# TimHarrelson/QuantumSimulations

Measured on AMD Instinct MI355X. Metric: detuning-points/hour (N=14 sea-detuning sweep, 3 variants per point), higher is better.
Workload: dtype f64 (complex128 state); 1 GPU; config 3: n_sea=13+1 rare (N=14 qubits), one 64-point sweep split over 1 GPU(s) (64 detunings in [0,150 kHz] x 3 variants = 192 evolutions on rank 0), t_final=0.001s, 101 outputs, 7 observables; propagator=exact Chebyshev (tol 1e-14), engine_mode=persistent, outputs_per_launch=2, parallelism=evolution-sharded x1 (strong scaling, no collectives), span_problems=0

## Files before the change

quantumsimulations_amd/csrc/dse_interval.hip:

```cpp
#include <type_traits>

#include "dse_device.h"

namespace dse {

#ifdef DSE_DIAG
__device__ int g_dse_ablate_iv = 0;
hipError_t set_ablate_interval(int mask) {
  return hipMemcpyToSymbol(HIP_SYMBOL(g_dse_ablate_iv), &mask, sizeof(int));
}
#else
constexpr int g_dse_ablate_iv = 0;
hipError_t set_ablate_interval(int mask) { return mask ? hipErrorNotSupported : hipSuccess; }
#endif

namespace {

typedef __attribute__((address_space(1))) int gint;


template <bool IMAG>
__device__ __forceinline__ double2 dmad(double2 acc, double cr, double ci, double2 s) {
  if (IMAG) {
    acc.x = fma(-ci, s.y, acc.x);
    acc.y = fma(ci, s.x, acc.y);
    return acc;
  }
  return cmad(acc, cr, ci, s);
}

__device__ __forceinline__ void rmad(double2& acc, double g, double2 s) {
  acc.x = fma(g, s.x, acc.x);
  acc.y = fma(g, s.y, acc.y);
}

typedef __attribute__((address_space(3))) const dv2 ldv2;

template <typename T>
__device__ __forceinline__ uint32_t lds_addr(const T* p) {
  return (uint32_t)(size_t)(const __attribute__((address_space(3))) T*)p;
}

template <int NT, int NH, int NR>
__device__ __forceinline__ void ld_rows(const double2* w, int t, int hh, int r0, double2* v) {
  uint32_t a = lds_addr(w + t);
  constexpr uint32_t HALF = (uint32_t)NH * NT * 16u;
  if (hh) {
    if (HALF >= 65536u)
      asm("v_add_u32_e32 %0, %1, %2" : "=v"(a) : "i"(HALF), "v"(a));
    else
      a += HALF;
  }
#pragma unroll
  for (int rr = 0; rr < NR; ++rr) {
    const dv2 d = *(ldv2*)(size_t)(a + (uint32_t)(r0 + rr) * NT * 16u);
    v[rr] = make_double2(d.x, d.y);
  }
}

template <int L>
struct IvShared {
  double2 w[RB<L>::T];
  double c[L + 1];
  double zz[L * L];
  double zr[kRegAmps];
  dv2 td[3][RB<L>::NT];
  double xg[kRegBits];
  double xq[RB<L>::TB];
  dv2 it[RB<L>::TB][8];
};

template <int L, bool IMAG>
__global__ void __launch_bounds__(RB<L>::NT)
k_interval(const DevProb* __restrict__ probs, const int2* __restrict__ items, int q, int set,
           int n_out, int* __restrict__ flags, int* __restrict__ err, HandoffKnobs hk, long colstride) {
  constexpr int NT = RB<L>::NT, R = kRegAmps, TB = RB<L>::TB, NH = R / 2;
  constexpr bool PIPE = DSE_PIPE && IMAG;
  constexpr uint32_t T = 1u << L;
  __shared__ IvShared<L> S;
  __shared__ int s_fail;

  if (__hip_atomic_load(err, __ATOMIC_RELAXED, __HIP_MEMORY_SCOPE_AGENT) != 0) return;
  const int2 it = items[blockIdx.x];
  const DevProb& P = probs[it.x];
  const uint32_t h = colstride ? 0u : (uint32_t)it.y;
  const size_t coff = colstride ? (size_t)it.y * (size_t)colstride : 0;
  const int tid = threadIdx.x;
  const bool pair = (P.n == L + 1);
  const bool xgen = pair && P.n_pairs_hi > 0;
  const int K = P.degree;
  const double s1 = P.s1;
  const uint32_t b_me = h & 1u, b_pa = b_me ^ 1u;

  constexpr uint32_t TBYTES = T * 16u;
  const __amdgpu_buffer_rsrc_t psi_me = tile_rsrc(P.buf[q ? 2 : 0] + coff + (h << L), TBYTES);
  const __amdgpu_buffer_rsrc_t psi_pa = tile_rsrc(P.buf[q ? 2 : 0] + ((h ^ 1u) << L), TBYTES);
  double2* const xs_me = P.xslots + ((size_t)h * kXSlots << L);
  double2* const xs_pa = P.xslots + ((size_t)(h ^ 1u) * kXSlots << L);
  const __amdgpu_buffer_rsrc_t acc_t = tile_rsrc(P.buf[q ? 0 : 2] + coff + (h << L), TBYTES);
  const uint32_t voff = (uint32_t)tid * 16u;
  const int lane = tid & 63;
  const int wave = __builtin_amdgcn_readfirstlane(tid >> 6);
  gint* flag_me = (gint*)flags + (2 * it.x + (int)h) * kIvWaves + wave;
  const gint* flag_pa = (const gint*)flags + (2 * it.x + (int)(h ^ 1u)) * kIvWaves + wave;

  const cptr<DPair> cph = cst(P.pairs_hi);
  const cptr<DFlip> cfh = cst(P.flips_hi);
  const double* crow = (const double*)coef_row(P, set, 0);
  const size_t rstride = 2 * (size_t)(P.kcap1 + 1);
  int dj[kMaxOut];
#pragma unroll
  for (int j = 0; j < kMaxOut; ++j) dj[j] = j < n_out ? (int)crow[j * rstride] : 0;

  const int ab = g_dse_ablate_iv;
  const bool fences = hk.fences != 0;

  if (tid == 0) s_fail = 0;
  {
    const gdbl* zz = gptr(P.zz);
    const int n = P.n;
    for (int e = tid; e < L * L; e += NT) {
      const int i = e / L, j = e % L;
      S.zz[e] = (j > i) ? zz[i * n + j] : 0.0;
    }
    tile_diag_coeffs<L>(P, h, P.beta, S.c, tid);
    static_assert(sizeof(DSweep) == 80 && sizeof(DPair) == 16, "iteration table layout");
    const gd2* psw = (const gd2*)P.sweeps;
    const gd2* ptt = (const gd2*)P.pairs_tt;
    for (int e = tid; e < 8 * TB; e += NT) {
      const int j = e >> 3, c = e & 7;
      dv2 v;
      v.x = v.y = 0.0;
      if (c < 4)
        v = psw[j * 5 + c];
      else if (4 * j + c - 4 < P.n_pairs_tt)
        v = ptt[4 * j + c - 4];
      S.it[j][c] = v;
    }
  }
#pragma unroll
  for (int r = 0; r < R; ++r) S.w[r * NT + tid] = bld(psi_me, voff, (uint32_t)(r * NT * 16));
  __syncthreads();
  if (tid < kRegAmps) {
    double v = 0.0;
    for (int a = 0; a < kRegBits; ++a)
      for (int b = a + 1; b < kRegBits; ++b)
        v += S.zz[(TB + a) * L + TB + b] * ((0.5 - ((tid >> a) & 1)) * (0.5 - ((tid >> b) & 1)));
    S.zr[tid] = v;
  }
  double zt = S.c[L];
  double hr[kRegBits];
#pragma unroll
  for (int i = 0; i < kRegBits; ++i) hr[i] = S.c[TB + i];
#pragma unroll 1
  for (int j = 0; j < TB; ++j) {
    const double sj = 0.5 - (double)((tid >> j) & 1);
    double a = S.c[j];
#pragma unroll 1
    for (int i = j + 1; i < TB; ++i) a += S.zz[j * L + i] * (0.5 - (double)((tid >> i) & 1));
    zt += a * sj;
#pragma unroll
    for (int i = 0; i < kRegBits; ++i) hr[i] += S.zz[j * L + TB + i] * sj;
  }
  static_assert(kRegBits == 4, "td packing");
  {
    dv2 v;
    v.x = zt, v.y = hr[0];
    S.td[0][tid] = v;
    v.x = hr[1], v.y = hr[2];
    S.td[1][tid] = v;
    v.x = hr[3], v.y = 0.0;
    S.td[2][tid] = v;
  }
  if (tid < kRegBits) {
    double g = 0.0;
    if (xgen)
      for (int p = 0; p < P.n_pairs_hi; ++p)
        if (cph[p].mask_lo == (1u << (TB + tid))) g = cph[p].g;
    S.xg[tid] = g;
  }
  if (tid < TB) {
    double g = 0.0;
    if (xgen)
      for (int p = 0; p < P.n_pairs_hi; ++p)
        if (cph[p].mask_lo == (1u << tid)) g = cph[p].g;
    S.xq[tid] = g;
  }
  __syncthreads();

  double2 prev[R];
#pragma unroll
  for (int r = 0; r < R; ++r) prev[r] = make_double2(0.0, 0.0);

  auto term_loop = [&](auto xg_tag) {
  constexpr bool xgen = decltype(xg_tag)::value;
  const bool xraw = pair && !xgen;
  for (int k = 1; k <= K; ++k) {
    double2 out[R];
    auto phase1 = [&]() {
      double2 own[R];
#pragma unroll
      for (int r = 0; r < R; ++r) own[r] = S.w[r * NT + tid];
      if (ab & (512 | 4)) {
#pragma unroll
        for (int r = 0; r < R; ++r) out[r] = own[r];
      } else {
        const dv2 t01 = S.td[0][tid], t23 = S.td[1][tid], t4 = S.td[2][tid];
        const double tdv[1 + kRegBits] = {t01.x, t01.y, t23.x, t23.y, t4.x};
#pragma unroll
        for (int r = 0; r < R; ++r) {
          double d = tdv[0] + S.zr[r];
#pragma unroll
          for (int i = 0; i < kRegBits; ++i) d += ((r >> i) & 1 ? -0.5 : 0.5) * tdv[1 + i];
          out[r].x = d * own[r].x;
          out[r].y = d * own[r].y;
        }
        if (P.rflip_mask) {
#pragma unroll
          for (int i = 0; i < kRegBits; ++i) {
            if (!((P.rflip_mask >> i) & 1)) continue;
            const double c0r = P.rflip[i][0], c0i = P.rflip[i][1], c1r = P.rflip[i][2], c1i = P.rflip[i][3];
#pragma unroll
            for (int r = 0; r < R; ++r) {
              const bool v = (r >> i) & 1;
              out[r] = dmad<IMAG>(out[r], v ? c1r : c0r, v ? c1i : c0i, own[r ^ (1 << i)]);
            }
          }
        }
#pragma unroll
        for (int a = 0; a < kRegBits; ++a)
#pragma unroll
          for (int b = a + 1; b < kRegBits; ++b) {
            const double g = P.rr_g[rr_index(a, b)];
            if (g == 0.0) continue;
#pragma unroll
            for (int r = 0; r < R; ++r) {
              if (((r >> a) ^ (r >> b)) & 1) continue;
              rmad(out[r], g, own[r ^ ((1 << a) | (1 << b))]);
            }
          }
      }
    };
    if constexpr (!xgen) phase1();
    __syncthreads();

    if (xgen && !(ab & 64)) {
      double2 u[R];
#pragma unroll
      for (int r = 0; r < R; ++r) u[r] = make_double2(0.0, 0.0);
#pragma unroll
      for (int hh = 0; hh < 2; ++hh) {
        double2 ow[NH];
        ld_rows<NT, NH, NH>(S.w, tid, hh, 0, ow);
        for (int f = 0; f < P.n_flips_hi; ++f) {
          const double cr = b_pa ? cfh[f].re1 : cfh[f].re0, ci = b_pa ? cfh[f].im1 : cfh[f].im0;
#pragma unroll
          for (int rr = 0; rr < NH; ++rr) u[hh * NH + rr] = cmad(u[hh * NH + rr], cr, ci, ow[rr]);
        }
#pragma unroll
        for (int i = 0; i < 3; ++i)
#pragma unroll
          for (int rr = 0; rr < NH; ++rr) {
            const double g = (((rr >> i) & 1u) == b_pa) ? S.xg[i] : 0.0;
            rmad(u[hh * NH + rr], g, ow[rr ^ (1 << i)]);
          }
        {
          const double g = ((uint32_t)(1 - hh) == b_pa) ? S.xg[3] : 0.0;
#pragma unroll
          for (int rr = 0; rr < NH; ++rr) rmad(u[(1 - hh) * NH + rr], g, ow[rr]);
        }
      }
      constexpr int JL = TB < 6 ? TB : 6;
      double2 ba[NH], bb[NH];
      ld_rows<NT, NH, NH>(S.w, tid ^ 1, 0, 0, ba);
#pragma unroll
      for (int j = 0; j < JL; ++j) {
        const double gj = ((uint32_t)((tid >> j) & 1) == b_pa) ? S.xq[j] : 0.0;
        ld_rows<NT, NH, NH>(S.w, tid ^ (1 << j), 1, 0, bb);
#pragma unroll
        for (int rr = 0; rr < NH; ++rr) rmad(u[rr], gj, ba[rr]);
        if (j + 1 < JL) ld_rows<NT, NH, NH>(S.w, tid ^ (1 << (j + 1)), 0, 0, ba);
#pragma unroll
        for (int rr = 0; rr < NH; ++rr) rmad(u[NH + rr], gj, bb[rr]);
      }
#pragma unroll
      for (int j = JL; j < TB; ++j) {
        if ((uint32_t)__builtin_amdgcn_readfirstlane((tid >> j) & 1) != b_pa) continue;
        const double gj = S.xq[j];
        ld_rows<NT, NH, NH>(S.w, tid ^ (1 << j), 0, 0, ba);
        ld_rows<NT, NH, NH>(S.w, tid ^ (1 << j), 1, 0, bb);
#pragma unroll
        for (int rr = 0; rr < NH; ++rr) rmad(u[rr], gj, ba[rr]);
#pragma unroll
        for (int rr = 0; rr < NH; ++rr) rmad(u[NH + rr], gj, bb[rr]);
      }
      const __amdgpu_buffer_rsrc_t dst = tile_rsrc(xs_me + ((size_t)((k - 1) % kXSlots) << L), TBYTES);
#pragma unroll
      for (int r = 0; r < R; ++r) bst<kSc1>(dst, voff, (uint32_t)(r * NT * 16), u[r]);
    }

    if constexpr (xgen) phase1();

    auto publish = [&]() {
      if (pair && !(ab & 64) && (xgen || k > 1)) {
        asm volatile("s_waitcnt vmcnt(0)" ::: "memory");
        if (lane == 0) {
          if (fences) {
            __builtin_amdgcn_fence(__ATOMIC_RELEASE, "agent");
            asm volatile("s_waitcnt vmcnt(0)" ::: "memory");
          }
          __hip_atomic_store(flag_me, k, __ATOMIC_RELAXED, __HIP_MEMORY_SCOPE_AGENT);
        }
      }
    };

    constexpr int J_PUB = TB / 2;

#pragma unroll 1
    for (int j = 0; j < ((ab & 512) ? 0 : TB); ++j) {
      if (j == J_PUB) publish();
      const int pt = tid ^ (1 << j);
      double2 pv[NH];
      if constexpr (PIPE) ld_rows<NT, NH, NH>(S.w, pt, 0, 0, pv);
      dv2 swv[4], ttv[4];
      {
        uint32_t ia;
        asm("v_mov_b32_e32 %0, %1" : "=v"(ia) : "s"(lds_addr(&S.it[j][0])));
#pragma unroll
        for (int e = 0; e < 4; ++e) swv[e] = *(ldv2*)(size_t)(ia + 16u * e);
#pragma unroll
        for (int e = 0; e < 4; ++e) ttv[e] = *(ldv2*)(size_t)(ia + 16u * (4 + e));
      }
      const int bj = (tid >> j) & 1;
      const double cr = bj ? swv[1].x : swv[0].x, ci = bj ? swv[1].y : swv[0].y;
      double g0[kRegBits], g1[kRegBits];
#pragma unroll
      for (int i = 0; i < kRegBits; ++i) {
        const double g = (i & 1) ? swv[2 + i / 2].y : swv[2 + i / 2].x;
        g0[i] = bj ? 0.0 : g;
        g1[i] = bj ? g : 0.0;
      }
      int tpt[4];
      double ge[4];
#pragma unroll
      for (int qq = 0; qq < 4; ++qq) {
        const uint32_t m = (uint32_t)__double_as_longlong(ttv[qq].x);
        tpt[qq] = tid ^ (int)m;
        ge[qq] = par32((uint32_t)tid & m) ? 0.0 : ttv[qq].y;
      }
      auto gsel = [&](int i, int bit) { return bit ? g1[i] : g0[i]; };
      auto sweep = [&](int hh, const double2* pv) {
        double2* oh = out + hh * NH;
#pragma unroll
        for (int rr = 0; rr < NH; ++rr) oh[rr] = dmad<IMAG>(oh[rr], cr, ci, pv[rr]);
#pragma unroll
        for (int i = 0; i < 3; ++i)
#pragma unroll
          for (int rr = 0; rr < NH; ++rr) rmad(oh[rr], gsel(i, (rr >> i) & 1), pv[rr ^ (1 << i)]);
        double2* oo = out + (1 - hh) * NH;
        const double g3 = gsel(3, 1 - hh);
#pragma unroll
        for (int rr = 0; rr < NH; ++rr) rmad(oo[rr], g3, pv[rr]);
      };
      auto tpair = [&](int qq, int hh, const double2* tv) {
        double2* oh = out + hh * NH;
#pragma unroll
        for (int rr = 0; rr < NH; ++rr) rmad(oh[rr], ge[qq], tv[rr]);
      };
      if constexpr (PIPE) {
        constexpr int NQ = NH / 2;
        auto tpair_q = [&](int qq, int hh, int qh, const double2* tv) {
          double2* oh = out + hh * NH + qh * NQ;
#pragma unroll
          for (int rr = 0; rr < NQ; ++rr) rmad(oh[rr], ge[qq], tv[rr]);
        };
        double2 qa[NQ], qb[NQ];
#pragma unroll
        for (int hh = 0; hh < 2; ++hh) {
          ld_rows<NT, NH, NQ>(S.w, tpt[0], hh, 0, qa);
          sweep(hh, pv);
#pragma unroll
          for (int qq = 0; qq < 4; ++qq) {
            ld_rows<NT, NH, NQ>(S.w, tpt[qq], hh, NQ, qb);
            tpair_q(qq, hh, 0, qa);
            if (qq < 3)
              ld_rows<NT, NH, NQ>(S.w, tpt[qq + 1], hh, 0, qa);
            else if (hh == 0)
              ld_rows<NT, NH, NH>(S.w, pt, 1, 0, pv);
            tpair_q(qq, hh, 1, qb);
          }
        }
      } else {
#pragma unroll
        for (int hh = 0; hh < 2; ++hh) {
          ld_rows<NT, NH, NH>(S.w, pt, hh, 0, pv);
          sweep(hh, pv);
#pragma unroll
          for (int qq = 0; qq < 4; ++qq) {
            double2 tv[NH];
            ld_rows<NT, NH, NH>(S.w, tpt[qq], hh, 0, tv);
            tpair(qq, hh, tv);
          }
        }
      }
    }
    if (ab & 512) publish();
    if (pair && !(ab & 128)) {
      const __amdgpu_buffer_rsrc_t src =
          (xraw && k == 1) ? psi_pa : tile_rsrc(xs_pa + ((size_t)((k - 1) % kXSlots) << L), TBYTES);
      double xr = 0.0, xi = 0.0;
      if (xraw && P.n_flips_hi > 0) {
        xr = b_me ? cfh[0].re1 : cfh[0].re0;
        xi = b_me ? cfh[0].im1 : cfh[0].im0;
      }
        if ((xgen || k > 1) && lane == 0 && !(ab & 64)) {
          int spins = 0;
          const int limit = hk.spin_limit;
          while (limit < 0 || __hip_atomic_load(flag_pa, __ATOMIC_RELAXED, __HIP_MEMORY_SCOPE_AGENT) < k) {
            __builtin_amdgcn_s_sleep(1);
            if (limit < 0 || ++spins > limit ||
                ((spins & 1023) == 0 && __hip_atomic_load(err, __ATOMIC_RELAXED, __HIP_MEMORY_SCOPE_AGENT))) {
              s_fail = 1;
              atomicExch(err, 1);
              break;
            }
          }
          if (fences) {
            __builtin_amdgcn_fence(__ATOMIC_ACQUIRE, "agent");
            asm volatile("s_waitcnt vmcnt(0)" ::: "memory");
          }
        }
      asm volatile("" ::: "memory");
#pragma unroll
      for (int hh = 0; hh < 2; ++hh) {
        double2 uv[NH];
#pragma unroll
        for (int rr = 0; rr < NH; ++rr) uv[rr] = bld<kSc1>(src, voff, (uint32_t)((hh * NH + rr) * NT * 16));
#pragma unroll
        for (int rr = 0; rr < NH; ++rr) {
          double2& o = out[hh * NH + rr];
          if (xgen) {
            o.x += uv[rr].x;
            o.y += uv[rr].y;
          } else {
            o = dmad<IMAG>(o, xr, xi, uv[rr]);
          }
        }
      }
    }

#pragma unroll
    for (int r = 0; r < R; ++r) {
      if (k == 1) {
        out[r].x *= s1;
        out[r].y *= s1;
      } else {
        out[r].x = fma(2.0 * s1, out[r].x, -prev[r].x);
        out[r].y = fma(2.0 * s1, out[r].y, -prev[r].y);
      }
    }
    constexpr int AB = kMaxOut <= 2 ? 4 : (kMaxOut == 3 ? 2 : 1);
    const int nj = (ab & 256) ? 0 : n_out;
    bool upd[kMaxOut];
    __amdgpu_buffer_rsrc_t acc_j[kMaxOut];
#pragma unroll
    for (int j = 0; j < kMaxOut; ++j) {
      upd[j] = j < nj && coef_nterm(k, dj[j]) > 0;
      acc_j[j] = (j == n_out - 1) ? acc_t
                                  : tile_rsrc(P.xacc + ((size_t)(q * P.xacc_q + j) << (L + P.tbl)) + (h << L), TBYTES);
    }
#pragma unroll
    for (int r0 = 0; r0 < R; r0 += AB) {
      double2 ownb[AB];
#pragma unroll
      for (int r = 0; r < AB; ++r) ownb[r] = S.w[(r0 + r) * NT + tid];
      double2 accv[kMaxOut][AB];
#pragma unroll
      for (int j = 0; j < kMaxOut; ++j)
        if (upd[j] && k > 1) {
#pragma unroll
          for (int r = 0; r < AB; ++r) accv[j][r] = bld(acc_j[j], voff, (uint32_t)((r0 + r) * NT * 16));
        }
#pragma unroll
      for (int j = 0; j < kMaxOut; ++j) {
        if (!upd[j]) continue;
        const int nt = coef_nterm(k, dj[j]);
        const auto cc = crow + j * rstride + 2 * (size_t)(k - 1);
        const double2 c0 = nt >= 3 ? make_double2(cc[0], cc[1]) : make_double2(0.0, 0.0),
                      c1 = nt >= 2 ? make_double2(cc[2], cc[3]) : make_double2(0.0, 0.0),
                      c2 = make_double2(cc[4], cc[5]);
#pragma unroll
        for (int r = 0; r < AB; ++r) {
          double2 a = make_double2(0.0, 0.0);
          if (k > 1) a = cmad(accv[j][r], c0.x, c0.y, prev[r0 + r]);
          a = cmad(a, c1.x, c1.y, ownb[r]);
          a = cmad(a, c2.x, c2.y, out[r0 + r]);
          bst(acc_j[j], voff, (uint32_t)((r0 + r) * NT * 16), a);
        }
      }
#pragma unroll
      for (int r = 0; r < AB; ++r) prev[r0 + r] = ownb[r];
    }
    __syncthreads();
    if (s_fail) break;
#pragma unroll
    for (int r = 0; r < R; ++r) S.w[r * NT + tid] = out[r];
    if (xraw && k < K && !(ab & 64)) {
      const __amdgpu_buffer_rsrc_t dst = tile_rsrc(xs_me + ((size_t)(k % kXSlots) << L), TBYTES);
#pragma unroll
      for (int r = 0; r < R; ++r) bst<kSc1>(dst, voff, (uint32_t)(r * NT * 16), out[r]);
    }
  }
  };
  if (xgen)
    term_loop(std::true_type{});
  else
    term_loop(std::false_type{});
}

__global__ void k_zero_flags(const int2* __restrict__ items, int n_items, int* __restrict__ flags) {
  const int i = blockIdx.x * blockDim.x + threadIdx.x;
  if (i < n_items * kIvWaves) {
    const int2 e = items[i / kIvWaves];
    flags[(2 * e.x + e.y) * kIvWaves + i % kIvWaves] = 0;
  }
}

}

hipError_t zero_flags(const int2* items, int n_items, int* flags, hipStream_t st) {
  if (n_items <= 0) return hipSuccess;
  hipLaunchKernelGGL(k_zero_flags, dim3((n_items * kIvWaves + 255) / 256), dim3(256), 0, st, items, n_items, flags);
  return hipGetLastError();
}

bool interval_supported(int L) { return L >= kRegBlockMinTile && L <= kMaxTile; }

hipError_t interval_occupancy(int L, bool imag, int* blocks_per_cu) {
  switch (L) {
#define X(l)                                                                                       \
  case l:                                                                                          \
    return imag ? hipOccupancyMaxActiveBlocksPerMultiprocessor(blocks_per_cu, k_interval<l, true>, \
                                                               RB<l>::NT, 0)                       \
                : hipOccupancyMaxActiveBlocksPerMultiprocessor(blocks_per_cu, k_interval<l, false>,\
                                                               RB<l>::NT, 0);
    X(10) X(11) X(12) X(13)
#undef X
    default:
      return hipErrorInvalidValue;
  }
}

hipError_t launch_interval(int L, bool imag, const DevProb* probs, const int2* items, int n_items,
                           int q, int set, int n_out, int* flags, int* err, HandoffKnobs hk, hipStream_t st,
                           long colstride) {
  if (n_items <= 0) return hipSuccess;
  switch (L) {
#define X(l)                                                                                     \
  case l:                                                                                        \
    if (imag)                                                                                    \
      hipLaunchKernelGGL((k_interval<l, true>), dim3(n_items), dim3(RB<l>::NT), 0, st, probs,  \
                         items, q, set, n_out, flags, err, hk, colstride);                        \
    else                                                                                         \
      hipLaunchKernelGGL((k_interval<l, false>), dim3(n_items), dim3(RB<l>::NT), 0, st, probs, \
                         items, q, set, n_out, flags, err, hk, colstride);                        \
    return hipGetLastError();
    X(10) X(11) X(12) X(13)
#undef X
    default:
      return hipErrorInvalidValue;
  }
}

}
```

Measured before the change: 862,900 detuning-points/hour.

## Fold Chebyshev output sums over rotating row groups with early-issued loads

Instead of updating every output accumulator row on every Chebyshev term, each term now folds only one of three row groups, picked by (k-1)%3. That group's accumulator rows are issued as loads before the partner-exchange wait so their latency overlaps the spin. Coefficients are loaded once per wave and broadcast with readlane instead of per-thread scalar loads. On the last term for an output, the remaining groups are folded with direct loads. The aim is to cut per-term global accumulator traffic and hide its latency, at the cost of a more complex schedule, more registers, and a dependency on coef_nterm taking a new phase argument whose definition is not shown.

```diff
diff --git a/quantumsimulations_amd/csrc/dse_interval.hip b/quantumsimulations_amd/csrc/dse_interval.hip
--- a/quantumsimulations_amd/csrc/dse_interval.hip
+++ b/quantumsimulations_amd/csrc/dse_interval.hip
@@ -32,6 +32,18 @@
 __device__ __forceinline__ void rmad(double2& acc, double g, double2 s) {
   acc.x = fma(g, s.x, acc.x);
   acc.y = fma(g, s.y, acc.y);
+}
+
+constexpr int kSumRows = 6;
+__host__ __device__ constexpr int sum_row0(int g) { return g == 0 ? 0 : (g == 1 ? 6 : 11); }
+static_assert(sum_row0(1) - sum_row0(0) <= kSumRows && sum_row0(2) - sum_row0(1) == kSumRows - 1 &&
+                  kRegAmps - sum_row0(2) == kSumRows - 1,
+              "the early loads take kSumRows - 1 rows, and one more for group 0");
+
+__device__ __forceinline__ double lane_value(double v, int l) {
+  const int lo = __builtin_amdgcn_readlane(__double2loint(v), l);
+  const int hi = __builtin_amdgcn_readlane(__double2hiint(v), l);
+  return __hiloint2double(hi, lo);
 }
 
 typedef __attribute__((address_space(3))) const dv2 ldv2;
@@ -110,7 +122,8 @@
   const size_t rstride = 2 * (size_t)(P.kcap1 + 1);
   int dj[kMaxOut];
 #pragma unroll
-  for (int j = 0; j < kMaxOut; ++j) dj[j] = j < n_out ? (int)crow[j * rstride] : 0;
+  for (int j = 0; j < kMaxOut; ++j)
+    dj[j] = j < n_out ? __builtin_amdgcn_readfirstlane((int)crow[j * rstride]) : 0;
 
   const int ab = g_dse_ablate_iv;
   const bool fences = hk.fences != 0;
@@ -287,8 +300,10 @@
       for (int j = JL; j < TB; ++j) {
         if ((uint32_t)__builtin_amdgcn_readfirstlane((tid >> j) & 1) != b_pa) continue;
         const double gj = S.xq[j];
-        ld_rows<NT, NH, NH>(S.w, tid ^ (1 << j), 0, 0, ba);
-        ld_rows<NT, NH, NH>(S.w, tid ^ (1 << j), 1, 0, bb);
+        int tq = tid;
+        asm volatile("" : "+v"(tq));
+        ld_rows<NT, NH, NH>(S.w, tq ^ (1 << j), 0, 0, ba);
+        ld_rows<NT, NH, NH>(S.w, tq ^ (1 << j), 1, 0, bb);
 #pragma unroll
         for (int rr = 0; rr < NH; ++rr) rmad(u[rr], gj, ba[rr]);
 #pragma unroll
@@ -405,6 +420,40 @@
       }
     }
     if (ab & 512) publish();
+
+    const int g = (k - 1) % 3;
+    const int nj = (ab & 256) ? 0 : n_out;
+    int ntj[kMaxOut];
+    __amdgpu_buffer_rsrc_t acc_j[kMaxOut];
+#pragma unroll
+    for (int j = 0; j < kMaxOut; ++j) {
+      ntj[j] = j < nj ? coef_nterm(k, dj[j], g) : 0;
+      acc_j[j] = (j == n_out - 1) ? acc_t
+                                  : tile_rsrc(P.xacc + ((size_t)(q * P.xacc_q + j) << (L + P.tbl)) + (h << L), TBYTES);
+    }
+    double2 accv[kMaxOut][kSumRows];
+#pragma unroll
+    for (int j = 0; j < kMaxOut; ++j)
+#pragma unroll
+      for (int r = 0; r < kSumRows; ++r) accv[j][r] = make_double2(0.0, 0.0);
+    double cv = 0.0;
+    if (k > 1) {
+      asm volatile("s_waitcnt vmcnt(0)" ::: "memory");
+      const uint32_t gso = (uint32_t)sum_row0(g) * NT * 16u;
+#pragma unroll
+      for (int j = 0; j < kMaxOut; ++j)
+        if (ntj[j] > 0) {
+#pragma unroll
+          for (int r = 0; r < kSumRows - 1; ++r) accv[j][r] = bld(acc_j[j], voff, gso + (uint32_t)(r * NT * 16));
+          if (g == 0) accv[j][kSumRows - 1] = bld(acc_j[j], voff, gso + (uint32_t)((kSumRows - 1) * NT * 16));
+        }
+      uint32_t lv = (uint32_t)tid;
+      asm volatile("" : "+v"(lv));
+      const uint32_t lj = (lv >> 3) & 7u, le = lv & 7u;
+      const uint32_t cj = lj < (uint32_t)nj ? lj : 0u, ce = le < 6u ? le : 5u;
+      cv = gptr(crow)[cj * rstride + 2 * (size_t)(k - 1) + ce];
+    }
+
     if (pair && !(ab & 128)) {
       const __amdgpu_buffer_rsrc_t src =
           (xraw && k == 1) ? psi_pa : tile_rsrc(xs_pa + ((size_t)((k - 1) % kXSlots) << L), TBYTES);
@@ -431,20 +480,16 @@
           }
         }
       asm volatile("" ::: "memory");
-#pragma unroll
-      for (int hh = 0; hh < 2; ++hh) {
-        double2 uv[NH];
-#pragma unroll
-        for (int rr = 0; rr < NH; ++rr) uv[rr] = bld<kSc1>(src, voff, (uint32_t)((hh * NH + rr) * NT * 16));
-#pragma unroll
-        for (int rr = 0; rr < NH; ++rr) {
-          double2& o = out[hh * NH + rr];
-          if (xgen) {
-            o.x += uv[rr].x;
-            o.y += uv[rr].y;
-          } else {
-            o = dmad<IMAG>(o, xr, xi, uv[rr]);
-          }
+      double2 uv[R];
+#pragma unroll
+      for (int r = 0; r < R; ++r) uv[r] = bld<kSc1>(src, voff, (uint32_t)(r * NT * 16));
+#pragma unroll
+      for (int r = 0; r < R; ++r) {
+        if (xgen) {
+          out[r].x += uv[r].x;
+          out[r].y += uv[r].y;
+        } else {
+          out[r] = dmad<IMAG>(out[r], xr, xi, uv[r]);
         }
       }
     }
@@ -459,48 +504,77 @@
         out[r].y = fma(2.0 * s1, out[r].y, -prev[r].y);
       }
     }
-    constexpr int AB = kMaxOut <= 2 ? 4 : (kMaxOut == 3 ? 2 : 1);
-    const int nj = (ab & 256) ? 0 : n_out;
-    bool upd[kMaxOut];
-    __amdgpu_buffer_rsrc_t acc_j[kMaxOut];
-#pragma unroll
-    for (int j = 0; j < kMaxOut; ++j) {
-      upd[j] = j < nj && coef_nterm(k, dj[j]) > 0;
-      acc_j[j] = (j == n_out - 1) ? acc_t
-                                  : tile_rsrc(P.xacc + ((size_t)(q * P.xacc_q + j) << (L + P.tbl)) + (h << L), TBYTES);
-    }
-#pragma unroll
-    for (int r0 = 0; r0 < R; r0 += AB) {
-      double2 ownb[AB];
-#pragma unroll
-      for (int r = 0; r < AB; ++r) ownb[r] = S.w[(r0 + r) * NT + tid];
-      double2 accv[kMaxOut][AB];
-#pragma unroll
-      for (int j = 0; j < kMaxOut; ++j)
-        if (upd[j] && k > 1) {
-#pragma unroll
-          for (int r = 0; r < AB; ++r) accv[j][r] = bld(acc_j[j], voff, (uint32_t)((r0 + r) * NT * 16));
-        }
+    double ccv[kMaxOut][6];
+#pragma unroll
+    for (int j = 0; j < kMaxOut; ++j)
+#pragma unroll
+      for (int e = 0; e < 6; ++e) ccv[j][e] = lane_value(cv, 8 * j + e);
+    auto fold = [&](auto r0_tag, auto nr_tag, auto src_tag, int ph) {
+      constexpr int R0 = decltype(r0_tag)::value, NR = decltype(nr_tag)::value, SRC = decltype(src_tag)::value;
+      double2 ownb[NR];
+#pragma unroll
+      for (int r = 0; r < NR; ++r) ownb[r] = S.w[(R0 + r) * NT + tid];
 #pragma unroll
       for (int j = 0; j < kMaxOut; ++j) {
-        if (!upd[j]) continue;
-        const int nt = coef_nterm(k, dj[j]);
-        const auto cc = crow + j * rstride + 2 * (size_t)(k - 1);
+        const int nt = j < nj ? coef_nterm(k, dj[j], ph) : 0;
+        if (nt == 0) continue;
+        double cc[6];
+        if constexpr (SRC == 1) {
+#pragma unroll
+          for (int e = 0; e < 6; ++e) cc[e] = ccv[j][e];
+        } else {
+          const gdbl* cg = gptr(crow) + j * rstride + 2 * (size_t)(k - 1);
+#pragma unroll
+          for (int e = 0; e < 6; ++e) cc[e] = cg[e];
+        }
         const double2 c0 = nt >= 3 ? make_double2(cc[0], cc[1]) : make_double2(0.0, 0.0),
                       c1 = nt >= 2 ? make_double2(cc[2], cc[3]) : make_double2(0.0, 0.0),
                       c2 = make_double2(cc[4], cc[5]);
-#pragma unroll
-        for (int r = 0; r < AB; ++r) {
+        double2 av[NR];
+        if constexpr (SRC == 2) {
+#pragma unroll
+          for (int r = 0; r < NR; ++r) av[r] = bld(acc_j[j], voff, (uint32_t)((R0 + r) * NT * 16));
+        }
+#pragma unroll
+        for (int r = 0; r < NR; ++r) {
           double2 a = make_double2(0.0, 0.0);
-          if (k > 1) a = cmad(accv[j][r], c0.x, c0.y, prev[r0 + r]);
+          if constexpr (SRC == 1) a = cmad(accv[j][r], c0.x, c0.y, prev[R0 + r]);
+          if constexpr (SRC == 2) a = cmad(av[r], c0.x, c0.y, prev[R0 + r]);
           a = cmad(a, c1.x, c1.y, ownb[r]);
-          a = cmad(a, c2.x, c2.y, out[r0 + r]);
-          bst(acc_j[j], voff, (uint32_t)((r0 + r) * NT * 16), a);
-        }
-      }
-#pragma unroll
-      for (int r = 0; r < AB; ++r) prev[r0 + r] = ownb[r];
-    }
+          a = cmad(a, c2.x, c2.y, out[R0 + r]);
+          bst(acc_j[j], voff, (uint32_t)((R0 + r) * NT * 16), a);
+        }
+      }
+    };
+    using std::integral_constant;
+    constexpr integral_constant<int, 0> i0{};
+    constexpr integral_constant<int, 1> i1{};
+    constexpr integral_constant<int, 2> i2{};
+    constexpr integral_constant<int, sum_row0(1)> g1r{};
+    constexpr integral_constant<int, sum_row0(2)> g2r{};
+    constexpr integral_constant<int, sum_row0(1) - sum_row0(0)> g0n{};
+    constexpr integral_constant<int, sum_row0(2) - sum_row0(1)> g1n{};
+    constexpr integral_constant<int, R - sum_row0(2)> g2n{};
+    if (k == 1) {
+      if (nj > 0) fold(i0, integral_constant<int, R>{}, i0, 0);
+    } else {
+      if (g == 0)
+        fold(i0, g0n, i1, 0);
+      else if (g == 1)
+        fold(g1r, g1n, i1, 1);
+      else
+        fold(g2r, g2n, i1, 2);
+      bool last = false;
+#pragma unroll
+      for (int j = 0; j < kMaxOut; ++j) last = last || (j < nj && dj[j] == k);
+      if (last) {
+        if (g != 0) fold(i0, g0n, i2, 0);
+        if (g != 1) fold(g1r, g1n, i2, 1);
+        if (g != 2) fold(g2r, g2n, i2, 2);
+      }
+    }
+#pragma unroll
+    for (int r = 0; r < R; ++r) prev[r] = S.w[r * NT + tid];
     __syncthreads();
     if (s_fail) break;
 #pragma unroll
```

Result: no change. 861,000 detuning-points/hour (-0.2%).
